# MarineRoboticsGroup/mac

Measured on AMD Instinct MI355X. Metric: frank_wolfe_iters_per_sec, higher is better.
Workload: dtype f64; 1 GPU; configs[3]: ER N=100000 ~2M candidates, chain fixed, K=10%; N=100000, m_candidates=2001737, K=200173, fixed_edges=99999, fw_iters=209, parallelism=single GPU

## Files before the change

mac_amd/csrc/kernels.h:

```cpp
#pragma once
#include <algorithm>

#include "common.h"

namespace machip {

template <typename T>
struct CsrViewT {
    int n;
    const int* rowptr;
    const int* col;
    const T* val;
};
using CsrView = CsrViewT<double>;

struct PatternView {
    int n;
    const int* prow;
    const int* pcol;
    const int* pk;
    const double* pw;
};

struct LanState {
// ... 39 lines not shown
    const int r1 = min(P.n, r0 + rows_per_block);
    int local = 0, supp = 0, mx = 0;
    for (int r = r0 + g; r < r1; r += GPB) {
        const int b = P.prow[r], e = P.prow[r + 1];
        int c = 0, sc = 0;
        for (int p = b + lane; p < e; p += G) {
            const int k = P.pk[p];
            const bool cand = k >= 0;
            const bool act = cand ? x_bit(xbits, k) : true;
            c += act;
            sc += (cand && act);
        }
        c = group_sum_i<G>(c);
        sc = group_sum_i<G>(sc);
        if (lane == 0) {
            cnt[r] = c + 1;
            local += c + 1;
            supp += sc;
            mx = max(mx, c + 1);
        }
    }
    const int tot = block_sum_i(local, sm);
    const int stot = block_sum_i(supp, sm);
#pragma unroll
    for (int o = 32; o > 0; o >>= 1) mx = max(mx, __shfl_xor(mx, o, kWave));
    __syncthreads();
    if ((threadIdx.x & 63) == 0) sm[threadIdx.x >> 6] = mx;
    __syncthreads();
    if (threadIdx.x == 0) {
        blk_sum[blockIdx.x] = tot;
        blk_sum[kAsmGrid + blockIdx.x] = stot;
        const int longest = max(max(sm[0], sm[1]), max(sm[2], sm[3]));
        blk_sum[2 * kAsmGrid + blockIdx.x] = longest;
        if (hsum) {
            hsum[blockIdx.x] = tot; hsum[kAsmGrid + blockIdx.x] = stot; hsum[2 * kAsmGrid + blockIdx.x] = longest;
        }
    }
}

struct PanSpec {
    int NP = 0;
    int C = 1;
    int band = 0;
    int* ps = nullptr;
    double* bd = nullptr;
    int* bpk = nullptr;
    int* ovf = nullptr;
};

template <int G>
__global__ __launch_bounds__(kBlock) void k_asm_fill(PatternView P, const unsigned int* __restrict__ xbits, const double* __restrict__ x,
                                                     int rows_per_block,
                                                     const int* __restrict__ cnt,
                                                     const int* __restrict__ blk_sum,
                                                     int* __restrict__ rowptr, int* __restrict__ col,
                                                     double* __restrict__ val,
                                                     double* __restrict__ blk_lnorm, PanSpec S = PanSpec()) {
    extern __shared__ __attribute__((aligned(16))) char smem_raw[];
    int* s_off = reinterpret_cast<int*>(smem_raw);
    __shared__ int sm_i[4];
    __shared__ double sm_d[4];
    __shared__ int s_chunk[kBlock];
    constexpr int GPB = kBlock / G;
    const int tid = threadIdx.x;
    const int lane = tid % G, g = tid / G;
    const int r0 = blockIdx.x * rows_per_block;
    const int r1 = min(P.n, r0 + rows_per_block);
    const int nr = max(0, r1 - r0);

// ... 1177 lines not shown
                                                     double tol = 0.0, unsigned long long* __restrict__ xbits_next = nullptr) {
#pragma clang fp contract(off)
    __shared__ double sm[4];
    const unsigned long long T = st->T;
    const long long lim = st->tie_limit;
    const bool none = st->k <= 0;
    double d = 0.0, q = 0.0;
    for (long i = (long)blockIdx.x * kBlock + threadIdx.x; i < m; i += (long)gridDim.x * kBlock) {
        const double gi = g[i];
        const unsigned long long key = f64_key(gi);
        const double s = (!none && (key > T || (key == T && (long long)i <= lim))) ? 1.0 : 0.0;
        if (s_out) s_out[i] = s;
        if (x) {
            const double xi = x[i];
            const double diff = s - xi;
            d += gi * diff;
            q += gi * gi;
            if (x_next) {
                const double step = gamma * diff;
                const double xn = xi + step;
                x_next[i] = xn;
                if (xbits_next) {
                    const unsigned long long bal = __ballot(xn > tol);
                    if ((threadIdx.x & 63) == 0) xbits_next[i >> 6] = bal;
                }
            }
        }
    }
    d = block_sum(d, sm);
    q = block_sum(q, sm);
    if (threadIdx.x == 0) { part[blockIdx.x] = d; part[kMaxGrid + blockIdx.x] = q; }
}

__global__ __launch_bounds__(kBlock) void k_round_keys(const double* __restrict__ x, long m, double f,
                                                       double* __restrict__ r) {
#pragma clang fp contract(off)
    for (long i = (long)blockIdx.x * kBlock + threadIdx.x; i < m; i += (long)gridDim.x * kBlock) {
        const double t = x[i] * f;
        r[i] = rint(t) / f;
    }
}
__global__ __launch_bounds__(kBlock) void k_tie_keys(const double* __restrict__ r, const double* __restrict__ cw,
                                                     long m, const SelState* __restrict__ st1,
                                                     double* __restrict__ keys2) {
    const unsigned long long T = st1->T;
    for (long i = (long)blockIdx.x * kBlock + threadIdx.x; i < m; i += (long)gridDim.x * kBlock)
        keys2[i] = f64_key(r[i]) == T ? cw[i] : -__builtin_huge_val();
}
__global__ __launch_bounds__(kBlock) void k_round_mark(const double* __restrict__ r, const double* __restrict__ keys2,
                                                       long m, const SelState* __restrict__ st1,
                                                       const SelState* __restrict__ st2, int two_level,
                                                       double* __restrict__ out) {
    const unsigned long long T1 = st1->T;
    const bool none = st1->k <= 0;
    for (long i = (long)blockIdx.x * kBlock + threadIdx.x; i < m; i += (long)gridDim.x * kBlock) {
        const unsigned long long k1 = f64_key(r[i]);
        bool sel = false;
        if (!none) {
            if (k1 > T1) sel = true;
            else if (k1 == T1) {
                if (!two_level) sel = (long long)i >= st1->tie_limit;
                else {
                    const unsigned long long k2 = f64_key(keys2[i]);
                    sel = k2 > st2->T || (k2 == st2->T && (long long)i >= st2->tie_limit);
                }
            }
// ... 54 lines not shown
```

mac_amd/csrc/machip.hip:

```cpp
#include <rccl/rccl.h>
#include <unistd.h>

#include <algorithm>
#include <atomic>
#include <cmath>
#include <chrono>
#include <condition_variable>
#include <functional>
#include <future>
#include <memory>
#include <mutex>
#include <numeric>
#include <thread>
#include <vector>

#include "solver.h"
#include "esp.h"
#include "esp_free.h"
#include "esp_tree.h"
#include "esp_select.h"
#include "esp_relax.h"
#include "esp_exchange.h"
#include "esp_exchange_edge.h"
#include "eig_exchange.h"
// ... 43 lines not shown
    bool broken = false;
    bool barrier() {
        std::unique_lock<std::mutex> lk(mu);
        if (broken) return false;
        const unsigned long gen = generation;
        if (++waiting == nranks) { waiting = 0; ++generation; cv.notify_all(); return true; }
        cv.wait(lk, [&] { return generation != gen || broken; });
        return !broken;
    }
    void abort() {
        std::lock_guard<std::mutex> lk(mu);
        broken = true;
        cv.notify_all();
    }
};

struct machip_problem {
    int device = 0;
    hipStream_t stream = nullptr;
    int n = 0;
    long m = 0, m_pad = 0;
    double tol_sel = 1e-10;
    int *prow = nullptr, *pcol = nullptr, *pk = nullptr;
    double* pw = nullptr;
    long P = 0;
    int asm_G = 16, asm_rpb = 1, asm_grid = 1;
    int *ci = nullptr, *cj = nullptr;
    double* cw = nullptr;
    double *x = nullptr, *x_next = nullptr, *g = nullptr, *s = nullptr, *scratch_m = nullptr;
    int *cnt = nullptr, *blk_sum = nullptr, *rowptr = nullptr, *col = nullptr;
    double *val = nullptr, *blk_lnorm = nullptr;
    unsigned long long *xb = nullptr, *xb_next = nullptr;
    bool xb_valid = false, xb_next_valid = false;
    long nnz = 0, support = 0;
    int maxlen = 0;
    double lnorm = 0.0;
    bool assembled = false, have_vec = false, csr_only = false;
    bool band_dups_ok = true;
    unsigned int* hist = nullptr;
    SelState* sel = nullptr;
    double* part_fw = nullptr;
    int* h_int = nullptr;
    double* h_dbl = nullptr;
    int* d_hint = nullptr;
    double* d_hdbl = nullptr;
    Solver sol;
    ncclComm_t comm = nullptr;
    std::shared_ptr<LocalGroup> lgroup;
    bool first_collective_pending = false;
    hipEvent_t ev_g0 = nullptr, ev_g1 = nullptr, ev_g2 = nullptr;
    bool ev_g_valid = false;
    std::unique_ptr<IpcGroup> ipcg;
    int rank = 0, nranks = 1;
    bool is_lane = false, lane_fw_ready = false;
    std::vector<machip_problem*> lanes;
    unsigned long start_version = 0;
    unsigned long seen_start_version = ~0ul;

    CsrView csr() const { return CsrView{n, rowptr, col, val}; }
    PatternView pattern() const { return PatternView{n, prow, pcol, pk, pw}; }
};

static int create_lane_stream(const Options& opt, int device, hipStream_t* out) {
    if (OPT(lane_queues, 0) == 0) {
        hipDeviceProp_t prop;
        if (hipGetDeviceProperties(&prop, device) == hipSuccess && prop.multiProcessorCount > 0) {
// ... 73 lines not shown
            int band_slots = 0;
            for (size_t q = (size_t)prow[(size_t)r]; q < pcol.size(); ++q) band_slots += (pcol[q] == r - 1 || pcol[q] == r + 1);
            if (band_slots > 7) p->band_dups_ok = false;
        }
        prow[(size_t)r + 1] = (int)pcol.size();
    }
    p->P = (long)pcol.size();
    ST_TRY(dev_alloc(&p->prow, (size_t)n + 1));
    ST_TRY(dev_alloc(&p->pcol, (size_t)p->P)); ST_TRY(dev_alloc(&p->pk, (size_t)p->P)); ST_TRY(dev_alloc(&p->pw, (size_t)p->P));
    HIP_TRY(hipMemcpyAsync(p->prow, prow.data(), sizeof(int) * ((size_t)n + 1), hipMemcpyHostToDevice, p->stream));
    if (p->P) {
        HIP_TRY(hipMemcpyAsync(p->pcol, pcol.data(), sizeof(int) * (size_t)p->P, hipMemcpyHostToDevice, p->stream));
        HIP_TRY(hipMemcpyAsync(p->pk, pk.data(), sizeof(int) * (size_t)p->P, hipMemcpyHostToDevice, p->stream));
        HIP_TRY(hipMemcpyAsync(p->pw, pw.data(), sizeof(double) * (size_t)p->P, hipMemcpyHostToDevice, p->stream));
    }
    HIP_TRY(hipStreamSynchronize(p->stream));
    const double mean = n ? (double)p->P / n : 1.0;
    int G = 4;
    while (G < 64 && G < mean * 0.75) G <<= 1;
    p->asm_G = OPT(asm_g, G);
    const int gpb = kBlock / p->asm_G;
    long nblk = std::min<long>(std::min(kAsmGrid, std::max(1, OPT(asm_maxgrid, kAsmGrid))), ((long)n + gpb - 1) / gpb);
    if (nblk < 1) nblk = 1;
    long rpb = ((long)n + nblk - 1) / nblk;
    rpb = (rpb + gpb - 1) / gpb * gpb;
    p->asm_rpb = (int)rpb;
    p->asm_grid = (int)(((long)n + rpb - 1) / rpb);
    if (p->asm_grid < 1) p->asm_grid = 1;
    if ((rpb + 1) * (long)sizeof(int) > 64 * 1024)
        return fail(MACHIP_BAD_ARG, "num_nodes above the supported 16.7 million (row-offset scan of the assembly kernel)");
    return MACHIP_OK;
}

template <int G>
void launch_asm(machip_problem* p, const PanSpec& S) {
    const PatternView P = p->pattern();
    const unsigned int* xb32 = reinterpret_cast<const unsigned int*>(p->xb);
    k_asm_count<G><<<p->asm_grid, kBlock, 0, p->stream>>>(P, xb32, p->asm_rpb, p->cnt, p->blk_sum, p->d_hint);
    const size_t lds = sizeof(int) * ((size_t)p->asm_rpb + 1);
    k_asm_fill<G><<<p->asm_grid, kBlock, lds, p->stream>>>(P, xb32, p->x, p->asm_rpb, p->cnt, p->blk_sum,
                                                           p->rowptr, p->col, p->val, p->d_hdbl, S);
}

int assemble(machip_problem* p) {
    if (p->csr_only) return fail(MACHIP_BAD_ARG, "handle wraps a caller CSR; nothing to assemble");
    PanSpec S;
    ST_TRY(p->sol.pan_spec_prepare(&S));
    if (!p->xb_valid) {
        const int grid = std::max(1, (int)std::min<long>(kMaxGrid, (p->m + kBlock - 1) / kBlock));
        k_x_bits<<<grid, kBlock, 0, p->stream>>>(p->x, p->m, p->tol_sel, p->xb);
        p->xb_valid = true;
    }
    switch (p->asm_G) {
        case 4: launch_asm<4>(p, S); break;
        case 8: launch_asm<8>(p, S); break;
        case 16: launch_asm<16>(p, S); break;
        case 32: launch_asm<32>(p, S); break;
        default: launch_asm<64>(p, S); break;
    }
    HIP_TRY(hipGetLastError());
    const int gb = p->asm_grid;
    HIP_TRY(hipStreamSynchronize(p->stream));
    long nnz = 0, supp = 0;
    int maxlen = 0;
    double ln = 0.0;
    for (int b = 0; b < gb; ++b) {
        nnz += p->h_int[b]; supp += p->h_int[kAsmGrid + b]; maxlen = std::max(maxlen, p->h_int[2 * kAsmGrid + b]);
        ln = std::max(ln, p->h_dbl[b]);
    }
    p->nnz = nnz; p->support = supp / 2; p->lnorm = ln; p->maxlen = maxlen;
    p->assembled = true;
    return MACHIP_OK;
}

int alloc_common(machip_problem* p, int vbudget_mb = 0) {
    ST_TRY(p->sol.init(p->n, p->stream, vbudget_mb));
    HIP_TRY(hipHostMalloc((void**)&p->h_int, sizeof(int) * 3 * kAsmGrid, hipHostMallocMapped));
    HIP_TRY(hipHostMalloc((void**)&p->h_dbl, sizeof(double) * std::max(4 * kMaxGrid, kAsmGrid), hipHostMallocMapped));
    HIP_TRY(hipHostGetDevicePointer((void**)&p->d_hint, p->h_int, 0));
    HIP_TRY(hipHostGetDevicePointer((void**)&p->d_hdbl, p->h_dbl, 0));
    return MACHIP_OK;
}

int select_on(machip_problem* p, const double* keys, long k, SelState* st, int prefer_high, bool hist0_done = false) {
    const Options& opt = p->sol.opt;
    return sel_launch(p->stream, keys, p->m, std::max(0l, std::min(k, p->m)), st, p->hist, prefer_high, OPT(sel_small, 1) != 0, hist0_done);
}

int select_topk(machip_problem* p, long k, bool hist0_done = false) { return select_on(p, p->g, k, p->sel, 0, hist0_done); }

void shard_plan(long m, int nranks, int rank, long* lo, long* hi, long* shard) {
    const long sh = nranks > 0 ? (m + nranks - 1) / nranks : m;
    *shard = sh;
    *lo = std::min(m, sh * rank);
    *hi = std::min(m, *lo + sh);
}

int local_allgather(machip_problem* p, long shard) {
    LocalGroup& G = *p->lgroup;
    HIP_TRY(hipStreamSynchronize(p->stream));
    if (!G.barrier()) return fail(MACHIP_RCCL_ERROR, "in-process communicator was shut down by another rank");
    for (int r = 0; r < G.nranks; ++r)
        if (r != p->rank)
            HIP_TRY(hipMemcpyAsync(p->g + shard * r, G.g[(size_t)r] + shard * r, sizeof(double) * (size_t)shard,
                                   hipMemcpyDeviceToDevice, p->stream));
    HIP_TRY(hipStreamSynchronize(p->stream));
    if (!G.barrier()) return fail(MACHIP_RCCL_ERROR, "in-process communicator was shut down by another rank");
    return MACHIP_OK;
}

int compute_gradient(machip_problem* p, bool have_vec_now = false, long fuse_k = -1, bool* fused = nullptr) {
    const Options& opt = p->sol.opt;
    if (!p->have_vec && !have_vec_now) return fail(MACHIP_BAD_ARG, "no Fiedler vector on the device: call machip_fiedler first");
    const long m = p->m;
    long lo = 0, hi = m, shard = m;
    if (p->nranks > 1) shard_plan(m, p->nranks, p->rank, &lo, &hi, &shard);
    const bool ipc_gather = p->nranks > 1 && !p->comm && p->ipcg;
    if (ipc_gather) {
        k_ipc_pubwait<<<1, 64, 0, p->stream>>>(p->ipcg->view, 3);
// ... 134 lines not shown
                  int64_t m, const int32_t* ci, const int32_t* cj, const double* cw, double min_sel_tol,
                  machip_problem** out) {
    if (!out) return fail(MACHIP_BAD_ARG, "out is NULL");
    *out = nullptr;
    if (n < 2 || n > 2000000000ll) return fail(MACHIP_BAD_ARG, "num_nodes must be in [2, 2e9]");
    if (n_fixed < 0 || m < 0 || m > 2000000000ll) return fail(MACHIP_BAD_ARG, "bad edge counts");
    if ((n_fixed && (!fi || !fj || !fw)) || (m && (!ci || !cj || !cw))) return fail(MACHIP_BAD_ARG, "NULL edge array");
    if (n_fixed + m < n - 1) return fail(MACHIP_BAD_ARG, "fewer than n-1 edges: no spanning tree possible");
    if ((double)(n_fixed + m) > 0.5 * (double)n * (double)(n - 1)) return fail(MACHIP_BAD_ARG, "more edges than the complete graph");
    if (machip_device_count() <= 0) return fail(MACHIP_NO_DEVICE, "no HIP device visible");
    HIP_TRY(hipSetDevice(device));
    machip_problem* p = new machip_problem();
    p->device = device;
    p->n = (int)n;
    p->m = (long)m;
    p->m_pad = (long)m;
    p->tol_sel = min_sel_tol;
    int st = MACHIP_OK;
    auto body = [&]() -> int {
        HIP_TRY(hipStreamCreateWithFlags(&p->stream, hipStreamNonBlocking));
        ST_TRY(build_pattern(p, n_fixed, fi, fj, fw, m, ci, cj, cw));
        const size_t mp = (size_t)m + 64 * 8;
        ST_TRY(dev_alloc(&p->ci, mp)); ST_TRY(dev_alloc(&p->cj, mp)); ST_TRY(dev_alloc(&p->cw, mp));
        ST_TRY(dev_alloc(&p->x, mp)); ST_TRY(dev_alloc(&p->x_next, mp)); ST_TRY(dev_alloc(&p->g, mp)); ST_TRY(dev_alloc(&p->s, mp));
        if (m) {
            HIP_TRY(hipMemcpyAsync(p->ci, ci, sizeof(int) * (size_t)m, hipMemcpyHostToDevice, p->stream));
            HIP_TRY(hipMemcpyAsync(p->cj, cj, sizeof(int) * (size_t)m, hipMemcpyHostToDevice, p->stream));
            HIP_TRY(hipMemcpyAsync(p->cw, cw, sizeof(double) * (size_t)m, hipMemcpyHostToDevice, p->stream));
        }
        HIP_TRY(hipMemsetAsync(p->x, 0, sizeof(double) * mp, p->stream));
        HIP_TRY(hipMemsetAsync(p->g, 0, sizeof(double) * mp, p->stream));
        HIP_TRY(hipStreamSynchronize(p->stream));
        const size_t cap = (size_t)p->P + (size_t)n + 8;
        ST_TRY(dev_alloc(&p->cnt, (size_t)n + 1)); ST_TRY(dev_alloc(&p->blk_sum, 3 * kAsmGrid));
        ST_TRY(dev_alloc(&p->rowptr, (size_t)n + 1)); ST_TRY(dev_alloc(&p->col, cap)); ST_TRY(dev_alloc(&p->val, cap));
        ST_TRY(dev_alloc(&p->blk_lnorm, kAsmGrid));
        ST_TRY(dev_alloc(&p->xb, (size_t)m / 64 + 2)); ST_TRY(dev_alloc(&p->xb_next, (size_t)m / 64 + 2));
        ST_TRY(dev_alloc(&p->hist, (6 + kSelRep) * kBins)); ST_TRY(dev_alloc(&p->sel, 2)); ST_TRY(dev_alloc(&p->part_fw, 2 * kMaxGrid));
        ST_TRY(alloc_common(p));
        p->sol.csr_cap = cap;
        p->sol.pat = p->pattern();
        p->sol.pan_allowed = p->band_dups_ok;
        {
            std::vector<char> has((size_t)n, 0);
            for (int64_t e = 0; e < n_fixed; ++e) {
                const int a = std::min(fi[e], fj[e]), b = std::max(fi[e], fj[e]);
                if (a >= 0 && b < n && b == a + 1 && fw[e] > 0.0) has[(size_t)a] = 1;
            }
            long cnt = 0;
            for (int64_t i = 0; i + 1 < n; ++i) cnt += has[(size_t)i];
            p->sol.chain_like = cnt >= (long)(0.98 * (double)(n - 1));
            p->sol.chain_edges = cnt;
        }
        return MACHIP_OK;
    };
    st = body();
    if (st != MACHIP_OK) { machip_destroy(p); return st; }
    *out = p;
    return MACHIP_OK;
}

void machip_destroy(machip_problem* p) {
    if (!p) return;
    for (machip_problem* q : p->lanes) machip_destroy(q);
    p->lanes.clear();
    (void)hipSetDevice(p->device);
    if (p->stream) (void)hipStreamSynchronize(p->stream);
    if (p->is_lane) { p->prow = p->pcol = p->pk = nullptr; p->pw = nullptr; p->ci = p->cj = nullptr; p->cw = nullptr; }
    if (p->comm) (void)ncclCommDestroy(p->comm);
    if (p->lgroup) p->lgroup->abort();
    if (p->ipcg) {
        IpcGroup& G = *p->ipcg;
        if (!G.clean_exit) { k_ipc_abort<<<1, 64, 0, p->stream>>>(G.view); (void)hipStreamSynchronize(p->stream); }
        p->sol.ipc = nullptr;
        p->ipcg.reset();
    }
    p->sol.destroy();
    void* ptrs[] = {p->prow, p->pcol, p->pk, p->pw, p->ci, p->cj, p->cw, p->x, p->x_next, p->g, p->s, p->scratch_m, p->cnt,
                    p->blk_sum, p->rowptr, p->col, p->val, p->blk_lnorm, p->xb, p->xb_next, p->hist, p->sel, p->part_fw};
    for (void* q : ptrs) if (q) (void)hipFree(q);
    for (hipEvent_t e : {p->ev_g0, p->ev_g1, p->ev_g2}) if (e) (void)hipEventDestroy(e);
    if (p->h_int) (void)hipHostFree(p->h_int);
    if (p->h_dbl) (void)hipHostFree(p->h_dbl);
    if (p->stream) (void)hipStreamDestroy(p->stream);
    delete p;
}

int machip_set_x(machip_problem* p, const double* x) {
    if (!p || !x || p->csr_only) return fail(MACHIP_BAD_ARG, "machip_set_x: bad handle or NULL x");
    HIP_TRY(hipSetDevice(p->device));
    HIP_TRY(hipMemcpyAsync(p->x, x, sizeof(double) * (size_t)p->m, hipMemcpyHostToDevice, p->stream));
    HIP_TRY(hipStreamSynchronize(p->stream));
    p->assembled = false; p->xb_valid = false;
    return MACHIP_OK;
}

int machip_get_x(machip_problem* p, double* x) {
    if (!p || !x || p->csr_only) return fail(MACHIP_BAD_ARG, "machip_get_x: bad handle or NULL x");
    HIP_TRY(hipSetDevice(p->device));
    HIP_TRY(hipMemcpyAsync(x, p->x, sizeof(double) * (size_t)p->m, hipMemcpyDeviceToHost, p->stream));
    HIP_TRY(hipStreamSynchronize(p->stream));
    return MACHIP_OK;
}

int machip_assemble(machip_problem* p, int64_t* nnz_out) {
    if (!p) return fail(MACHIP_BAD_ARG, "NULL handle");
    HIP_TRY(hipSetDevice(p->device));
    ST_TRY(assemble(p));
    if (nnz_out) *nnz_out = p->nnz;
    return MACHIP_OK;
}

int machip_get_laplacian(machip_problem* p, int32_t* indptr, int32_t* indices, double* data) {
    if (!p || !indptr || !indices || !data) return fail(MACHIP_BAD_ARG, "NULL argument");
    HIP_TRY(hipSetDevice(p->device));
    if (!p->assembled) ST_TRY(assemble(p));
    HIP_TRY(hipMemcpyAsync(indptr, p->rowptr, sizeof(int) * ((size_t)p->n + 1), hipMemcpyDeviceToHost, p->stream));
    HIP_TRY(hipMemcpyAsync(indices, p->col, sizeof(int) * (size_t)p->nnz, hipMemcpyDeviceToHost, p->stream));
    HIP_TRY(hipMemcpyAsync(data, p->val, sizeof(double) * (size_t)p->nnz, hipMemcpyDeviceToHost, p->stream));
    HIP_TRY(hipStreamSynchronize(p->stream));
    return MACHIP_OK;
}

int machip_fiedler(machip_problem* p, double tol, int max_steps, const double* x0, int warm_start,
                   double* lambda2, double* v_out, double* X_out, int q, machip_solve_stats* stats) {
    if (!p || !lambda2) return fail(MACHIP_BAD_ARG, "NULL argument");
// ... 40 lines not shown
    ST_TRY(compute_gradient(p));
    if (g_out) HIP_TRY(hipMemcpyAsync(g_out, p->g, sizeof(double) * (size_t)p->m, hipMemcpyDeviceToHost, p->stream));
    HIP_TRY(hipStreamSynchronize(p->stream));
    guard.ok = true;
    return MACHIP_OK;
}

int machip_lp_topk(machip_problem* p, int64_t k, double* s_out) {
    if (!p || p->csr_only) return fail(MACHIP_BAD_ARG, "bad handle");
    HIP_TRY(hipSetDevice(p->device));
    ST_TRY(select_topk(p, (long)k));
    const int grid = (int)std::min<long>(kMaxGrid, (p->m + kBlock - 1) / kBlock);
    k_fw_final<<<std::max(grid, 1), kBlock, 0, p->stream>>>(p->g, nullptr, p->m, p->sel, 0.0, nullptr, p->s, p->part_fw);
    if (s_out) HIP_TRY(hipMemcpyAsync(s_out, p->s, sizeof(double) * (size_t)p->m, hipMemcpyDeviceToHost, p->stream));
    HIP_TRY(hipStreamSynchronize(p->stream));
    return MACHIP_OK;
}

int machip_fw_step(machip_problem* p, int64_t k, int iter, double tol, int max_steps, int warm_start,
                   double* f, double* dual, double* gnorm, machip_solve_stats* stats) {
    if (!p || p->csr_only || !f || !dual || !gnorm) return fail(MACHIP_BAD_ARG, "bad argument");
    GroupGuard guard{p};
    HIP_TRY(hipSetDevice(p->device));
    ST_TRY(assemble(p));
    double lam = 0.0;
    const int grid = std::max(1, (int)std::min<long>(kMaxGrid, (p->m + kBlock - 1) / kBlock));
    const double gamma = 2.0 / ((double)iter + 2.0);
    int epi_status = MACHIP_OK;
    auto epilogue = [&](bool speculative) {
        bool fused = false;
        int st = compute_gradient(p, speculative, (long)k, &fused);
        if (st == MACHIP_OK) st = select_topk(p, (long)k, fused);
        if (st == MACHIP_OK) {
            k_fw_final<<<grid, kBlock, 0, p->stream>>>(p->g, p->x, p->m, p->sel, gamma, p->x_next, nullptr, p->d_hdbl, p->tol_sel, p->xb_next);
            p->xb_next_valid = true;
            if (hipGetLastError() != hipSuccess) st = fail(MACHIP_HIP_ERROR, "k_fw_final launch failed");
        }
        epi_status = st;
    };
    bool done = false;
    auto soft = [](int st) { return st == MACHIP_NOT_CONVERGED || st == MACHIP_DISCONNECTED; };
    if (p->lgroup && p->lgroup->shard_eig) {
        const int st = group_fiedler(p, tol, max_steps, warm_start, &lam, stats);
        if (st != MACHIP_OK) { guard.ok = soft(st); return st; }
    } else {
        const bool spec = p->nranks <= 1 && p->sol.opt.get(kOpt_spec_epilogue, 1) != 0;
        if (spec) p->sol.after_check = [&] { epilogue(true); };
        const int st = run_fiedler(p, tol, max_steps, nullptr, warm_start, &lam, stats);
        p->sol.after_check = nullptr;
        if (st != MACHIP_OK) { guard.ok = soft(st); return st; }
        done = spec && p->sol.hook_seq == p->sol.final_check_seq && epi_status == MACHIP_OK;
    }
    if (!done) {
        epilogue(false);
        if (epi_status != MACHIP_OK) return epi_status;
        HIP_TRY(hipStreamSynchronize(p->stream));
    }
    if (p->ipcg) ST_TRY(p->sol.ipc_check_err("gradient exchange"));
    double d = 0.0, q2 = 0.0;
    for (int b = 0; b < grid; ++b) { d += p->h_dbl[b]; q2 += p->h_dbl[kMaxGrid + b]; }
    *f = lam;
    *dual = lam + d;
    *gnorm = std::sqrt(q2);
    guard.ok = true;
    return MACHIP_OK;
}

int machip_fw_run(machip_problem* p, int64_t k, int first_iter, int max_iters, double gap_tol, double grad_tol, double tol, int max_steps,
                  int warm_start, double* upper_inout, double* f_traj, double* dual_traj, double* gnorm_traj, machip_solve_stats* stats,
// ... 27 lines not shown
    if (!p || p->csr_only || !rounded_out) return fail(MACHIP_BAD_ARG, "bad argument");
    if (decimals > 15) return fail(MACHIP_BAD_ARG, "decimals must be <= 15");
    HIP_TRY(hipSetDevice(p->device));
    const long m = p->m;
    if (m == 0) return MACHIP_OK;
    if (!p->scratch_m) ST_TRY(dev_alloc(&p->scratch_m, (size_t)m + 64));
    const int grid = std::max(1, (int)std::min<long>(kMaxGrid, (m + kBlock - 1) / kBlock));
    double* r = p->s;
    const bool tb = decimals >= 0;
    if (tb) k_round_keys<<<grid, kBlock, 0, p->stream>>>(p->x, m, std::pow(10.0, decimals), r);
    else HIP_TRY(hipMemcpyAsync(r, p->x, sizeof(double) * (size_t)m, hipMemcpyDeviceToDevice, p->stream));
    ST_TRY(select_on(p, r, (long)k, p->sel, 1));
    int two = 0;
    if (tb && k > 0 && k < m) {
        SelState h;
        HIP_TRY(hipMemcpyAsync(&h, p->sel, sizeof(SelState), hipMemcpyDeviceToHost, p->stream));
        HIP_TRY(hipStreamSynchronize(p->stream));
        if (h.kk < h.cnt_eq) {
            k_tie_keys<<<grid, kBlock, 0, p->stream>>>(r, p->cw, m, p->sel, p->scratch_m);
            ST_TRY(select_on(p, p->scratch_m, (long)h.kk, p->sel + 1, 1));
            two = 1;
        }
    }
    k_round_mark<<<grid, kBlock, 0, p->stream>>>(r, p->scratch_m, m, p->sel, p->sel + 1, two, r);
    HIP_TRY(hipMemcpyAsync(rounded_out, r, sizeof(double) * (size_t)m, hipMemcpyDeviceToHost, p->stream));
    HIP_TRY(hipStreamSynchronize(p->stream));
    return MACHIP_OK;
}

int machip_fw_commit(machip_problem* p) {
    if (!p || p->csr_only) return fail(MACHIP_BAD_ARG, "bad handle");
    std::swap(p->x, p->x_next);
    std::swap(p->xb, p->xb_next);
    p->xb_valid = p->xb_next_valid; p->xb_next_valid = false;
    p->assembled = false;
    return MACHIP_OK;
}

int machip_fiedler_csr(int device, int64_t n, const int32_t* indptr, const int32_t* indices, const double* data,
                       double tol, int max_steps, const double* x0, double* lambda2, double* v_out, double* X_out,
                       int q, machip_solve_stats* stats) {
    if (!indptr || !indices || !data || !lambda2) return fail(MACHIP_BAD_ARG, "NULL argument");
    if (n < 2 || n > 2000000000ll) return fail(MACHIP_BAD_ARG, "n must be in [2, 2e9]");
    if (X_out && (q < 1 || q > 4)) return fail(MACHIP_BAD_ARG, "q must be in [1,4]");
    const long nnz = indptr[n];
    if (indptr[0] != 0 || nnz < 0) return fail(MACHIP_BAD_ARG, "bad indptr: indptr[0] must be 0 and indptr[n] >= 0 (int32 row pointers: nnz < 2^31)");
    for (int64_t r = 0; r < n; ++r)
        if (indptr[r + 1] < indptr[r]) return fail(MACHIP_BAD_ARG, "indptr not monotone");
    double lnorm = 0.0;
    int maxlen_csr = 0;
    long chain_cnt = 0;
    for (int64_t r = 0; r < n; ++r) {
        double s = 0.0;
        for (long pp = indptr[r]; pp < (long)indptr[r + 1]; ++pp) {
            if (indices[pp] < 0 || indices[pp] >= n) return fail(MACHIP_BAD_ARG, "column index out of range");
            s += std::fabs(data[pp]);
            if (indices[pp] == r + 1 && data[pp] != 0.0) ++chain_cnt;
        }
        lnorm = std::max(lnorm, s);
        maxlen_csr = std::max(maxlen_csr, (int)(indptr[r + 1] - indptr[r]));
    }
    if (machip_device_count() <= 0) return fail(MACHIP_NO_DEVICE, "no HIP device visible");
    HIP_TRY(hipSetDevice(device));
    std::unique_lock<std::mutex> lk(g_csr_mu, std::try_to_lock);
    machip_problem* p = nullptr;
    bool cached = false;
// ... 297 lines not shown
}

#ifdef PAN_CLOCKS
extern "C" int machip_debug_pan_clocks(machip_problem* p, long long* out, int groups) {
    if (!p || !out || groups < 1 || groups > kMaxGrid || !p->sol.panv.clk) return fail(MACHIP_BAD_ARG, "machip_debug_pan_clocks: no clock buffer");
    HIP_TRY(hipSetDevice(p->device));
    HIP_TRY(hipStreamSynchronize(p->stream));
    HIP_TRY(hipMemcpy(out, p->sol.panv.clk, sizeof(long long) * 16 * (size_t)groups, hipMemcpyDeviceToHost));
    HIP_TRY(hipMemset(p->sol.panv.clk, 0, sizeof(long long) * 16 * (size_t)kMaxGrid));
    return MACHIP_OK;
}
#endif

int machip_shard_plan(int64_t m, int nranks, int rank, int64_t* lo, int64_t* hi, int64_t* shard) {
    if (m < 0 || nranks < 1 || rank < 0 || rank >= nranks || !lo || !hi || !shard) return fail(MACHIP_BAD_ARG, "machip_shard_plan: bad argument");
    long a, b, c;
    shard_plan((long)m, nranks, rank, &a, &b, &c);
    *lo = a; *hi = b; *shard = c;
    return MACHIP_OK;
}

namespace {
int make_lane(machip_problem* p, machip_problem** out) {
    machip_problem* q = new machip_problem();
    q->is_lane = true;
    q->device = p->device; q->n = p->n; q->m = p->m; q->m_pad = p->m; q->tol_sel = p->tol_sel;
    q->prow = p->prow; q->pcol = p->pcol; q->pk = p->pk; q->pw = p->pw; q->P = p->P;
    q->asm_G = p->asm_G; q->asm_rpb = p->asm_rpb; q->asm_grid = p->asm_grid;
    q->ci = p->ci; q->cj = p->cj; q->cw = p->cw;
    auto body = [&]() -> int {
        ST_TRY(create_lane_stream(p->sol.opt, q->device, &q->stream));
        ST_TRY(dev_alloc(&q->x, (size_t)q->m + 64));
        const size_t cap = (size_t)q->P + (size_t)q->n + 8;
        ST_TRY(dev_alloc(&q->cnt, (size_t)q->n + 1)); ST_TRY(dev_alloc(&q->blk_sum, 3 * kAsmGrid));
        ST_TRY(dev_alloc(&q->rowptr, (size_t)q->n + 1)); ST_TRY(dev_alloc(&q->col, cap)); ST_TRY(dev_alloc(&q->val, cap));
        ST_TRY(dev_alloc(&q->blk_lnorm, kAsmGrid));
        ST_TRY(dev_alloc(&q->xb, (size_t)q->m / 64 + 2)); ST_TRY(dev_alloc(&q->xb_next, (size_t)q->m / 64 + 2));
        const Options& opt = p->sol.opt;
        q->sol.opt = opt;
        ST_TRY(alloc_common(q, std::max(16, OPT(lane_vbudget_mb, std::max(16, OPT(vbudget_mb, 4096) / 8)))));
        q->sol.csr_cap = cap;
        q->sol.pat = q->pattern();
        q->sol.pan_allowed = p->sol.pan_allowed;
        q->sol.chain_like = p->sol.chain_like; q->sol.chain_edges = p->sol.chain_edges;
        return MACHIP_OK;
    };
    const int st = body();
    if (st != MACHIP_OK) { machip_destroy(q); return st; }
    *out = q;
    return MACHIP_OK;
}

int ensure_lane_fw(machip_problem* q) {
    if (q->lane_fw_ready) return MACHIP_OK;
    const size_t mp = (size_t)q->m + 64 * 8;
    if (!q->x_next) ST_TRY(dev_alloc(&q->x_next, mp));
    if (!q->g) ST_TRY(dev_alloc(&q->g, mp));
    if (!q->s) ST_TRY(dev_alloc(&q->s, mp));
    if (!q->hist) ST_TRY(dev_alloc(&q->hist, (6 + kSelRep) * kBins));
    if (!q->sel) ST_TRY(dev_alloc(&q->sel, 2));
    if (!q->part_fw) ST_TRY(dev_alloc(&q->part_fw, 2 * kMaxGrid));
    HIP_TRY(hipMemsetAsync(q->g, 0, sizeof(double) * mp, q->stream));
    HIP_TRY(hipStreamSynchronize(q->stream));
    q->lane_fw_ready = true;
    return MACHIP_OK;
}

// ... 20 lines not shown
        q->sol.throughput_lane = true;
        if (p->sol.have_start && q->seen_start_version != p->start_version) {
            HIP_TRY(hipMemcpyAsync(q->sol.start, p->sol.start, sizeof(double) * (size_t)p->n, hipMemcpyDeviceToDevice, q->stream));
            HIP_TRY(hipStreamSynchronize(q->stream));
            q->sol.have_start = true;
            q->seen_start_version = p->start_version;
        }
    }
    if (fw) for (int l = 0; l < nl; ++l) ST_TRY(ensure_lane_fw(p->lanes[(size_t)l]));
    *nl_out = nl;
    return MACHIP_OK;
}
}

int machip_eval_batch(machip_problem* p, int B, const double* X, double tol, int max_steps, double* lambda2, int* status) {
    if (!p || p->csr_only || p->is_lane || B < 0 || (B && (!X || !lambda2))) return fail(MACHIP_BAD_ARG, "machip_eval_batch: bad argument");
    if (B == 0) return MACHIP_OK;
    HIP_TRY(hipSetDevice(p->device));
    int nl = 0;
    ST_TRY(prepare_lanes(p, B, false, &nl));
    std::atomic<int> next{0};
    std::vector<int> lane_status((size_t)nl, MACHIP_OK);
    std::vector<std::string> lane_err((size_t)nl);
    auto work = [&](int l) {
        machip_problem* q = p->lanes[(size_t)l];
        if (hipSetDevice(q->device) != hipSuccess) { lane_status[(size_t)l] = MACHIP_HIP_ERROR; lane_err[(size_t)l] = "hipSetDevice failed"; return; }
        for (int b = next.fetch_add(1); b < B; b = next.fetch_add(1)) {
            int st = MACHIP_OK;
            double lam = 0.0;
            if (hipMemcpyAsync(q->x, X + (size_t)b * (size_t)q->m, sizeof(double) * (size_t)q->m, hipMemcpyHostToDevice, q->stream) != hipSuccess ||
                hipStreamSynchronize(q->stream) != hipSuccess) {
                st = fail(MACHIP_HIP_ERROR, "machip_eval_batch: copy of x failed");
            } else {
                q->assembled = false; q->xb_valid = false;
                st = assemble(q);
                q->sol.have_prev = false; q->sol.warm_skip = 0; q->sol.warm_fails = 0; q->sol.last_pr = 0.0; q->sol.hist_lan_steps = -1; q->sol.hist_lob_iters = -1; q->sol.hist_exact_iters = -1; q->sol.last_steps = 0; q->sol.last_steps_lowp = 0;
                if (st == MACHIP_OK) st = run_fiedler(q, tol, max_steps, nullptr, 0, &lam, nullptr);
            }
            lambda2[b] = lam;
            if (status) status[b] = st;
            if (st != MACHIP_OK && st != MACHIP_NOT_CONVERGED && st != MACHIP_DISCONNECTED) {
                lane_status[(size_t)l] = st; lane_err[(size_t)l] = g_err;
                return;
            }
        }
    };
    std::vector<std::thread> th;
    for (int l = 1; l < nl; ++l) th.emplace_back(work, l);
    work(0);
    for (auto& t : th) t.join();
    for (int l = 0; l < nl; ++l)
        if (lane_status[(size_t)l] != MACHIP_OK) return fail((machip_status)lane_status[(size_t)l], lane_err[(size_t)l]);
    return MACHIP_OK;
}

int machip_fw_sweep(machip_problem* p, int B, const int64_t* ks, const double* X0, int max_iters, double gap_tol,
                    double grad_tol, double tol, int max_steps, int warm_start, int round_decimals, double* X_out,
                    double* R_out, double* upper, double* f_traj, int* iters, int* status) {
    if (!p || p->csr_only || p->is_lane || B < 0 || max_iters < 0 || (B && (!ks || !X0 || !X_out || !upper || !iters || !status)))
        return fail(MACHIP_BAD_ARG, "machip_fw_sweep: bad argument");
    if (p->nranks > 1) return fail(MACHIP_BAD_ARG, "machip_fw_sweep: not on a handle that belongs to a communicator");
    if (B == 0) return MACHIP_OK;
    HIP_TRY(hipSetDevice(p->device));
    int nl = 0;
    ST_TRY(prepare_lanes(p, B, true, &nl));
    const size_t m = (size_t)p->m;
    std::atomic<int> next{0};
// ... 414 lines not shown
```

mac_amd/csrc/options.h:

```cpp
#pragma once
#include <climits>
#include <cstdlib>
#include <cstring>
#include <mutex>
#include <string>

namespace machip {

#define MACHIP_OPTION_LIST(X)                                                                                                      \
                                                                                                          \
    X(solver) X(graph) X(debug) X(chunk) X(chunk_near) X(sched) X(near_x10) X(trigger_pct) X(classic_n) X(persist) X(pchunk)      \
    X(spec_epilogue) X(spec_slack_pct) X(f32_switch_e9) X(tailless) X(stream) X(stream_trigger_pct) X(stream_retry_pct) X(stream_look) X(stream_margin) X(stream_window) X(stream_far) X(start_land) X(start_pow) X(start_floor_e6) X(start_land_pr_permille) X(start_land_min_mean10)                                                                \
                                                                        \
    X(spmv) X(g) X(unroll) X(block) X(maxgrid) X(defer) X(tpr) X(ell)                                                              \
                                                                                                            \
    X(panel) X(panel_min_n) X(panel_min_mean10) X(panel_multi_min_mean10) X(panel_np) X(panel_nb) X(panel_b2) X(panel_g2)         \
    X(panel_cells) X(panel_maxcells) X(panel_band) X(panel_u) X(panel_u_amp) X(pan32) X(pan32_switch_e9) X(panel_ops) X(panel_rev)                                                                               \
                                                                                                 \
    X(woodbury) X(wb_max) X(wb_hard) X(wb_lane_max) X(exact_big) X(exact_switch) X(gj_look_min) X(lob_density_pct) X(lob_chunk)   \
    X(lob_patience) X(lob_small_s) X(lob_fuse)                                                                                     \
     \
    X(sel_small) X(sel_fuse) X(asm_g) X(asm_maxgrid) X(vbudget_mb) X(vcap) X(lanes) X(lane_vbudget_mb) X(lane_queues) X(shard_eig) X(ipc_panel) \
    X(rccl_timeout_s)                                                                                                              \
               \
    X(esp_free_split)                                                                                                              \
       \
    X(esp_xch_lds_kb) X(esp_xch_max_mb) X(esp_xch_profile)                                                                         \
                                                       \
    X(eig_xch_max_mb)                                                                                                              \
                                                                                                            \
    X(eig_free_rows) X(eig_free_split)

enum OptId {
#define X(n) kOpt_##n,
    MACHIP_OPTION_LIST(X)
#undef X
    kNumOpts
};

constexpr long kOptAuto = LONG_MIN;

inline const char* const* option_names() {
    static const char* const names[] = {
#define X(n) #n,
        MACHIP_OPTION_LIST(X)
#undef X
        nullptr};
    return names;
}
inline int option_id(const char* name) {
    if (!name) return -1;
    const char* const* nm = option_names();
    for (int i = 0; i < kNumOpts; ++i) if (!strcmp(nm[i], name)) return i;
    return -1;
}
// ... 44 lines not shown
```

Measured before the change: 133.3 iter/s.

## Carry per-row degree counts across FW iterations instead of recounting in assembly

The Frank-Wolfe update kernel now compares each candidate's new support bit against the old one and atomically adjusts the per-node degree counts for edges that flip. The next assembly then skips the full pattern count pass and runs a light totals kernel that only re-sums the carried counts per block. This targets the cost of rescanning the whole pattern every iteration, at the price of atomics in the update kernel and state tracking of count validity across swaps and resets. The path can be disabled with an option.

```diff
diff --git a/mac_amd/csrc/kernels.h b/mac_amd/csrc/kernels.h
--- a/mac_amd/csrc/kernels.h
+++ b/mac_amd/csrc/kernels.h
@@ -95,9 +95,45 @@
         blk_sum[kAsmGrid + blockIdx.x] = stot;
         const int longest = max(max(sm[0], sm[1]), max(sm[2], sm[3]));
         blk_sum[2 * kAsmGrid + blockIdx.x] = longest;
+        blk_sum[3 * kAsmGrid + blockIdx.x] = tot - stot;
         if (hsum) {
             hsum[blockIdx.x] = tot; hsum[kAsmGrid + blockIdx.x] = stot; hsum[2 * kAsmGrid + blockIdx.x] = longest;
         }
+    }
+}
+
+constexpr int kAsmTotalsGrid = 256;
+__global__ __launch_bounds__(kBlock) void k_asm_totals(int n, int rows_per_block, int nblk, const int* __restrict__ cnt,
+                                                       int* __restrict__ blk_sum, int* __restrict__ hsum) {
+    __shared__ int sm[3][4];
+    const int ln = threadIdx.x & 63, wv = threadIdx.x >> 6;
+    int wtot = 0, wstot = 0, wmx = 0;
+    for (int b = blockIdx.x * 4 + wv; b < nblk; b += gridDim.x * 4) {
+        const int r0 = b * rows_per_block;
+        const int r1 = min(n, r0 + rows_per_block);
+        int local = 0, mx = 0;
+        for (int r = r0 + ln; r < r1; r += 64) {
+            const int c = cnt[r];
+            local += c;
+            mx = max(mx, c);
+        }
+        local = group_sum_i<64>(local);
+#pragma unroll
+        for (int o = 32; o > 0; o >>= 1) mx = max(mx, __shfl_xor(mx, o, kWave));
+        if (ln == 0) {
+            const int stot = local - blk_sum[3 * kAsmGrid + b];
+            blk_sum[b] = local;
+            blk_sum[kAsmGrid + b] = stot;
+            blk_sum[2 * kAsmGrid + b] = mx;
+            wtot += local; wstot += stot; wmx = max(wmx, mx);
+        }
+    }
+    if (ln == 0) { sm[0][wv] = wtot; sm[1][wv] = wstot; sm[2][wv] = wmx; }
+    __syncthreads();
+    if (threadIdx.x == 0) {
+        hsum[blockIdx.x] = (sm[0][0] + sm[0][1]) + (sm[0][2] + sm[0][3]);
+        hsum[kAsmGrid + blockIdx.x] = (sm[1][0] + sm[1][1]) + (sm[1][2] + sm[1][3]);
+        hsum[2 * kAsmGrid + blockIdx.x] = max(max(sm[2][0], sm[2][1]), max(sm[2][2], sm[2][3]));
     }
 }
 
@@ -1341,6 +1377,62 @@
     if (threadIdx.x == 0) { part[blockIdx.x] = d; part[kMaxGrid + blockIdx.x] = q; }
 }
 
+__global__ __launch_bounds__(kBlock) void k_fw_final_carry(const double* __restrict__ g, const double* __restrict__ x,
+                                                           long m, const SelState* __restrict__ st, double gamma,
+                                                           double* __restrict__ x_next, double* __restrict__ part ,
+                                                           double tol, unsigned long long* xbits_next, const unsigned long long* xbits_old,
+                                                           int* __restrict__ cnt, const int* __restrict__ ci, const int* __restrict__ cj) {
+#pragma clang fp contract(off)
+    __shared__ double sm[4];
+    const unsigned long long T = st->T;
+    const long long lim = st->tie_limit;
+    const bool none = st->k <= 0;
+    const int ln = threadIdx.x & 63;
+    const long stride = (long)gridDim.x * kBlock;
+    double d = 0.0, q = 0.0;
+    long i = (long)blockIdx.x * kBlock + threadIdx.x;
+    double gi = 0.0, xi = 0.0;
+    unsigned long long oldw = 0;
+    if (i < m) {
+        gi = g[i]; xi = x[i];
+        if (ln == 0) oldw = xbits_old[i >> 6];
+    }
+    int pa = 0, pb = 0, pd = 0;
+    while (i < m) {
+        if (pd) {
+            if (pa != pb) { atomicAdd(&cnt[pa], pd); atomicAdd(&cnt[pb], pd); }
+            pd = 0;
+        }
+        const long in = i + stride;
+        double gn = 0.0, xn1 = 0.0;
+        unsigned long long oldn = 0;
+        if (in < m) {
+            gn = g[in]; xn1 = x[in];
+            if (ln == 0) oldn = xbits_old[in >> 6];
+        }
+        const unsigned long long key = f64_key(gi);
+        const double s = (!none && (key > T || (key == T && (long long)i <= lim))) ? 1.0 : 0.0;
+        const double diff = s - xi;
+        d += gi * diff;
+        q += gi * gi;
+        const double step = gamma * diff;
+        const double xn = xi + step;
+        x_next[i] = xn;
+        const bool on = xn > tol;
+        const unsigned long long bal = __ballot(on);
+        const unsigned int lo = __builtin_amdgcn_readfirstlane((unsigned int)oldw);
+        const unsigned int hi = __builtin_amdgcn_readfirstlane((unsigned int)(oldw >> 32));
+        const bool was = ((ln < 32 ? lo >> ln : hi >> (ln - 32)) & 1u) != 0;
+        if (ln == 0) xbits_next[i >> 6] = bal;
+        if (was != on) { pa = ci[i]; pb = cj[i]; pd = on ? 1 : -1; }
+        i = in; gi = gn; xi = xn1; oldw = oldn;
+    }
+    if (pd && pa != pb) { atomicAdd(&cnt[pa], pd); atomicAdd(&cnt[pb], pd); }
+    d = block_sum(d, sm);
+    q = block_sum(q, sm);
+    if (threadIdx.x == 0) { part[blockIdx.x] = d; part[kMaxGrid + blockIdx.x] = q; }
+}
+
 __global__ __launch_bounds__(kBlock) void k_round_keys(const double* __restrict__ x, long m, double f,
                                                        double* __restrict__ r) {
 #pragma clang fp contract(off)
diff --git a/mac_amd/csrc/machip.hip b/mac_amd/csrc/machip.hip
--- a/mac_amd/csrc/machip.hip
+++ b/mac_amd/csrc/machip.hip
@@ -99,6 +99,8 @@
     double *val = nullptr, *blk_lnorm = nullptr;
     unsigned long long *xb = nullptr, *xb_next = nullptr;
     bool xb_valid = false, xb_next_valid = false;
+    enum CntOf { kCntNone, kCntCur, kCntNext };
+    CntOf cnt_of = kCntNone;
     long nnz = 0, support = 0;
     int maxlen = 0;
     double lnorm = 0.0;
@@ -238,11 +240,14 @@
     return MACHIP_OK;
 }
 
+int asm_totals_grid(const machip_problem* p) { return std::min(kAsmTotalsGrid, (p->asm_grid + 3) / 4); }
+
 template <int G>
-void launch_asm(machip_problem* p, const PanSpec& S) {
+void launch_asm(machip_problem* p, const PanSpec& S, bool carried) {
     const PatternView P = p->pattern();
     const unsigned int* xb32 = reinterpret_cast<const unsigned int*>(p->xb);
-    k_asm_count<G><<<p->asm_grid, kBlock, 0, p->stream>>>(P, xb32, p->asm_rpb, p->cnt, p->blk_sum, p->d_hint);
+    if (carried) k_asm_totals<<<asm_totals_grid(p), kBlock, 0, p->stream>>>(p->n, p->asm_rpb, p->asm_grid, p->cnt, p->blk_sum, p->d_hint);
+    else k_asm_count<G><<<p->asm_grid, kBlock, 0, p->stream>>>(P, xb32, p->asm_rpb, p->cnt, p->blk_sum, p->d_hint);
     const size_t lds = sizeof(int) * ((size_t)p->asm_rpb + 1);
     k_asm_fill<G><<<p->asm_grid, kBlock, lds, p->stream>>>(P, xb32, p->x, p->asm_rpb, p->cnt, p->blk_sum,
                                                            p->rowptr, p->col, p->val, p->d_hdbl, S);
@@ -256,24 +261,27 @@
         const int grid = std::max(1, (int)std::min<long>(kMaxGrid, (p->m + kBlock - 1) / kBlock));
         k_x_bits<<<grid, kBlock, 0, p->stream>>>(p->x, p->m, p->tol_sel, p->xb);
         p->xb_valid = true;
-    }
+        p->cnt_of = machip_problem::kCntNone;
+    }
+    const bool carried = p->cnt_of == machip_problem::kCntCur && p->sol.opt.get(kOpt_asm_carry, 1) != 0;
+    p->cnt_of = machip_problem::kCntNone;
     switch (p->asm_G) {
-        case 4: launch_asm<4>(p, S); break;
-        case 8: launch_asm<8>(p, S); break;
-        case 16: launch_asm<16>(p, S); break;
-        case 32: launch_asm<32>(p, S); break;
-        default: launch_asm<64>(p, S); break;
+        case 4: launch_asm<4>(p, S, carried); break;
+        case 8: launch_asm<8>(p, S, carried); break;
+        case 16: launch_asm<16>(p, S, carried); break;
+        case 32: launch_asm<32>(p, S, carried); break;
+        default: launch_asm<64>(p, S, carried); break;
     }
     HIP_TRY(hipGetLastError());
+    p->cnt_of = machip_problem::kCntCur;
     const int gb = p->asm_grid;
+    const int gi = carried ? asm_totals_grid(p) : gb;
     HIP_TRY(hipStreamSynchronize(p->stream));
     long nnz = 0, supp = 0;
     int maxlen = 0;
     double ln = 0.0;
-    for (int b = 0; b < gb; ++b) {
-        nnz += p->h_int[b]; supp += p->h_int[kAsmGrid + b]; maxlen = std::max(maxlen, p->h_int[2 * kAsmGrid + b]);
-        ln = std::max(ln, p->h_dbl[b]);
-    }
+    for (int b = 0; b < gi; ++b) { nnz += p->h_int[b]; supp += p->h_int[kAsmGrid + b]; maxlen = std::max(maxlen, p->h_int[2 * kAsmGrid + b]); }
+    for (int b = 0; b < gb; ++b) ln = std::max(ln, p->h_dbl[b]);
     p->nnz = nnz; p->support = supp / 2; p->lnorm = ln; p->maxlen = maxlen;
     p->assembled = true;
     return MACHIP_OK;
@@ -291,6 +299,14 @@
 int select_on(machip_problem* p, const double* keys, long k, SelState* st, int prefer_high, bool hist0_done = false) {
     const Options& opt = p->sol.opt;
     return sel_launch(p->stream, keys, p->m, std::max(0l, std::min(k, p->m)), st, p->hist, prefer_high, OPT(sel_small, 1) != 0, hist0_done);
+}
+
+const unsigned long long* carry_from(machip_problem* p) {
+    if (p->sol.opt.get(kOpt_asm_carry, 1) == 0 || (p->cnt_of == machip_problem::kCntCur && !p->xb_valid)) p->cnt_of = machip_problem::kCntNone;
+    if (p->cnt_of == machip_problem::kCntNone) return nullptr;
+    const unsigned long long* from = p->cnt_of == machip_problem::kCntCur ? p->xb : p->xb_next;
+    p->cnt_of = machip_problem::kCntNext;
+    return from;
 }
 
 int select_topk(machip_problem* p, long k, bool hist0_done = false) { return select_on(p, p->g, k, p->sel, 0, hist0_done); }
@@ -491,7 +507,7 @@
         HIP_TRY(hipMemsetAsync(p->g, 0, sizeof(double) * mp, p->stream));
         HIP_TRY(hipStreamSynchronize(p->stream));
         const size_t cap = (size_t)p->P + (size_t)n + 8;
-        ST_TRY(dev_alloc(&p->cnt, (size_t)n + 1)); ST_TRY(dev_alloc(&p->blk_sum, 3 * kAsmGrid));
+        ST_TRY(dev_alloc(&p->cnt, (size_t)n + 1)); ST_TRY(dev_alloc(&p->blk_sum, 4 * kAsmGrid));
         ST_TRY(dev_alloc(&p->rowptr, (size_t)n + 1)); ST_TRY(dev_alloc(&p->col, cap)); ST_TRY(dev_alloc(&p->val, cap));
         ST_TRY(dev_alloc(&p->blk_lnorm, kAsmGrid));
         ST_TRY(dev_alloc(&p->xb, (size_t)m / 64 + 2)); ST_TRY(dev_alloc(&p->xb_next, (size_t)m / 64 + 2));
@@ -550,7 +566,7 @@
     HIP_TRY(hipSetDevice(p->device));
     HIP_TRY(hipMemcpyAsync(p->x, x, sizeof(double) * (size_t)p->m, hipMemcpyHostToDevice, p->stream));
     HIP_TRY(hipStreamSynchronize(p->stream));
-    p->assembled = false; p->xb_valid = false;
+    p->assembled = false; p->xb_valid = false; p->cnt_of = machip_problem::kCntNone;
     return MACHIP_OK;
 }
 
@@ -657,9 +673,12 @@
         int st = compute_gradient(p, speculative, (long)k, &fused);
         if (st == MACHIP_OK) st = select_topk(p, (long)k, fused);
         if (st == MACHIP_OK) {
-            k_fw_final<<<grid, kBlock, 0, p->stream>>>(p->g, p->x, p->m, p->sel, gamma, p->x_next, nullptr, p->d_hdbl, p->tol_sel, p->xb_next);
+            const unsigned long long* from = carry_from(p);
+            if (from) k_fw_final_carry<<<grid, kBlock, 0, p->stream>>>(p->g, p->x, p->m, p->sel, gamma, p->x_next, p->d_hdbl, p->tol_sel, p->xb_next,
+                                                                       from, p->cnt, p->ci, p->cj);
+            else k_fw_final<<<grid, kBlock, 0, p->stream>>>(p->g, p->x, p->m, p->sel, gamma, p->x_next, nullptr, p->d_hdbl, p->tol_sel, p->xb_next);
             p->xb_next_valid = true;
-            if (hipGetLastError() != hipSuccess) st = fail(MACHIP_HIP_ERROR, "k_fw_final launch failed");
+            if (hipGetLastError() != hipSuccess) { p->cnt_of = machip_problem::kCntNone; st = fail(MACHIP_HIP_ERROR, "k_fw_final launch failed"); }
         }
         epi_status = st;
     };
@@ -753,6 +772,7 @@
     if (!p || p->csr_only) return fail(MACHIP_BAD_ARG, "bad handle");
     std::swap(p->x, p->x_next);
     std::swap(p->xb, p->xb_next);
+    p->cnt_of = (p->cnt_of == machip_problem::kCntNext && p->xb_next_valid) ? machip_problem::kCntCur : machip_problem::kCntNone;
     p->xb_valid = p->xb_next_valid; p->xb_next_valid = false;
     p->assembled = false;
     return MACHIP_OK;
@@ -1116,7 +1136,7 @@
         ST_TRY(create_lane_stream(p->sol.opt, q->device, &q->stream));
         ST_TRY(dev_alloc(&q->x, (size_t)q->m + 64));
         const size_t cap = (size_t)q->P + (size_t)q->n + 8;
-        ST_TRY(dev_alloc(&q->cnt, (size_t)q->n + 1)); ST_TRY(dev_alloc(&q->blk_sum, 3 * kAsmGrid));
+        ST_TRY(dev_alloc(&q->cnt, (size_t)q->n + 1)); ST_TRY(dev_alloc(&q->blk_sum, 4 * kAsmGrid));
         ST_TRY(dev_alloc(&q->rowptr, (size_t)q->n + 1)); ST_TRY(dev_alloc(&q->col, cap)); ST_TRY(dev_alloc(&q->val, cap));
         ST_TRY(dev_alloc(&q->blk_lnorm, kAsmGrid));
         ST_TRY(dev_alloc(&q->xb, (size_t)q->m / 64 + 2)); ST_TRY(dev_alloc(&q->xb_next, (size_t)q->m / 64 + 2));
@@ -1203,7 +1223,7 @@
                 hipStreamSynchronize(q->stream) != hipSuccess) {
                 st = fail(MACHIP_HIP_ERROR, "machip_eval_batch: copy of x failed");
             } else {
-                q->assembled = false; q->xb_valid = false;
+                q->assembled = false; q->xb_valid = false; q->cnt_of = machip_problem::kCntNone;
                 st = assemble(q);
                 q->sol.have_prev = false; q->sol.warm_skip = 0; q->sol.warm_fails = 0; q->sol.last_pr = 0.0; q->sol.hist_lan_steps = -1; q->sol.hist_lob_iters = -1; q->sol.hist_exact_iters = -1; q->sol.last_steps = 0; q->sol.last_steps_lowp = 0;
                 if (st == MACHIP_OK) st = run_fiedler(q, tol, max_steps, nullptr, 0, &lam, nullptr);
diff --git a/mac_amd/csrc/options.h b/mac_amd/csrc/options.h
--- a/mac_amd/csrc/options.h
+++ b/mac_amd/csrc/options.h
@@ -20,7 +20,7 @@
     X(woodbury) X(wb_max) X(wb_hard) X(wb_lane_max) X(exact_big) X(exact_switch) X(gj_look_min) X(lob_density_pct) X(lob_chunk)   \
     X(lob_patience) X(lob_small_s) X(lob_fuse)                                                                                     \
      \
-    X(sel_small) X(sel_fuse) X(asm_g) X(asm_maxgrid) X(vbudget_mb) X(vcap) X(lanes) X(lane_vbudget_mb) X(lane_queues) X(shard_eig) X(ipc_panel) \
+    X(sel_small) X(sel_fuse) X(asm_g) X(asm_maxgrid) X(asm_carry) X(vbudget_mb) X(vcap) X(lanes) X(lane_vbudget_mb) X(lane_queues) X(shard_eig) X(ipc_panel) \
     X(rccl_timeout_s)                                                                                                              \
                \
     X(esp_free_split)                                                                                                              \
```

Result: no change. 134.1 iter/s (median of 4 runs) (+0.6%).
